# CoderWZW/ARLib

Hardware: AMD Instinct MI355X
Metric: BPR-train interactions/sec (LightGCN d=64 L=3 + BPR + Adam, B=2048) (higher is better)
Workload: dtype f32

## Files before the change

### arlib_amd/_lib.py

```python
import ctypes as C
import os

_HERE = os.path.dirname(os.path.abspath(__file__))
LIB_PATH = os.environ.get('ARLIB_AMD_LIB') or os.path.join(_HERE, 'lib', 'libarlib_amd.so')
ABI_VERSION = 28
_lib = None


class ArlError(RuntimeError):
    pass


class arl_csr(C.Structure):
    _fields_ = [('n_rows', C.c_int64), ('nnz', C.c_int64), ('rowptr', C.c_void_p), ('col', C.c_void_p), ('val', C.c_void_p),
                ('chunk', C.c_int32), ('n_chunks', C.c_int64), ('chunk_row', C.c_void_p), ('chunk_begin', C.c_void_p),
                ('chunk_end', C.c_void_p), ('n_long', C.c_int64), ('long_row', C.c_void_p), ('long_first', C.c_void_p),
                ('long_count', C.c_void_p), ('partial', C.c_void_p), ('row_tasks', C.c_void_p)]


class arl_blocked(C.Structure):
    _fields_ = [('n_waves', C.c_int64), ('rows_per_wave', C.c_int64), ('loads_in_flight', C.c_int64), ('wave_ptr', C.c_void_p), ('wave_rows', C.c_void_p), ('rec_col', C.c_void_p),
                ('rec_val', C.c_void_p), ('n_split', C.c_int64), ('split_row', C.c_void_p), ('split_first', C.c_void_p), ('split_count', C.c_void_p),
                ('partial', C.c_void_p), ('waves_per_group', C.c_int64)]

# ... 6 lines not shown

_vp, _i64, _i32, _f = C.c_void_p, C.c_int64, C.c_int32, C.c_float
_SIGS = {
    'arl_abi_version': (C.c_int, []),
    'arl_mt_seed': (C.c_int, [_vp, _vp, _i64]),
    'arl_sampler_shuffle': (C.c_int, [_vp, _vp, _i64]),
    'arl_mt_sample_range': (C.c_int, [_vp, _i64, _i64, C.c_int32, _vp, _vp]),
    'arl_sampler_next_batch': (C.c_int, [_vp, _vp, _i64, _i64, _i32, _vp, _vp, _i64, _vp, _vp, _vp]),
    'arl_norm_adj_values_f32': (C.c_int, [_i64, _vp, _vp, _vp, _vp, _vp, _vp]),
    'arl_norm_adj_values_coo_f32': (C.c_int, [_i64, _vp, _vp, _vp, _vp, _i64, _vp, _vp, _vp]),
    'arl_norm_vals_coo_f32': (C.c_int, [_vp, _vp, _vp, _i64, _vp, _vp, _vp]),
    'arl_spmm_csr_f32': (C.c_int, [C.POINTER(arl_csr), _vp, _i64, _f, _f, _vp, _vp, _vp]),
    'arl_spmm_csr_layersum_f32': (C.c_int, [C.POINTER(arl_csr), _vp, _i64, _vp, _vp, _vp, _vp]),
    'arl_spmm_csr_adam_f32': (C.c_int, [C.POINTER(arl_csr), _vp, _i64, _f, _f, _vp, _vp, _vp, _vp, _vp, _f, _f, _f, _f, _i64, _vp]),
    'arl_spmm_blocked_f32': (C.c_int, [C.POINTER(arl_blocked), _vp, _i64, _f, _f, _vp, _vp, _vp, _vp]),
    'arl_spmm_csr_rscale_f32': (C.c_int, [C.POINTER(arl_csr), _vp, _i64, _vp, _f, _f, _vp, _vp, _vp]),
    'arl_spmm_blocked_rscale_f32': (C.c_int, [C.POINTER(arl_blocked), _vp, _i64, _vp, _f, _f, _vp, _vp, _vp]),
    'arl_spmm_blocked_layersum_f32': (C.c_int, [C.POINTER(arl_blocked), _vp, _i64, _vp, _vp, _vp, _vp]),
    'arl_spmm_blocked_adam_f32': (C.c_int, [C.POINTER(arl_blocked), _vp, _i64, _f, _f, _vp, _vp, _vp, _vp, _vp, _f, _f, _f, _f, _i64, _vp]),
    'arl_lpt_deal': (C.c_int, [_i64, _vp, _i64, _i64, _vp, _vp]),
    'arl_syn_v1_pairs': (_i64, [_i64, _i64, C.c_double, C.c_uint64, C.c_double, _i64, _i64, _vp, _i64]),
    'arl_graph_digest': (C.c_uint64, [_vp, _i64]),
    'arl_spmm_tiled_f32': (C.c_int, [C.POINTER(arl_tiled), _vp, _i64, _f, _f, _vp, _vp, _vp, _vp]),
    'arl_spmm_tiled_adam_f32': (C.c_int, [C.POINTER(arl_tiled), _vp, _i64, _f, _f, _vp, _vp, _vp, _vp, _vp, _f, _f, _f, _f, _i64, _vp]),
    'arl_spmm_csr_flagged_f32': (C.c_int, [C.POINTER(arl_csr), _vp, _i64, _vp, _f, _f, _vp, _vp, _vp, _vp]),
    'arl_spmm_csr_rows_workspace_bytes': (_i64, [_i64, _i64, _i64]),
    'arl_spmm_csr_rows_f32': (C.c_int, [C.POINTER(arl_csr), _vp, _i64, _vp, _i64, _i64, _vp, _i64, _f, _vp, _vp, _vp, _vp]),
    'arl_mark_rows_u8': (C.c_int, [_vp, _vp, _i64, _i32, _vp]),
    'arl_mark_rows_bits_u32': (C.c_int, [_vp, _vp, _i64, _i32, _vp]),
    'arl_zero_rows_f32': (C.c_int, [_vp, _vp, _i64, _i64, _vp]),
    'arl_batch_rows_set_f32': (C.c_int, [_vp, _vp, _vp, _vp, _i64, _i64, _vp, _f, _vp, _vp, _vp]),
    'arl_batch_rows_clear_f32': (C.c_int, [_vp, _vp, _vp, _vp, _i64, _i64, _vp, _vp]),
    'arl_bpr_l2_workspace_bytes': (_i64, [_i64]),
    'arl_bpr_l2_fwd_bwd_f32': (C.c_int, [_vp, _i64, _i64, _vp, _vp, _vp, _i64, _f, _f, _vp, _vp, _vp, _i32, _vp]),
    'arl_bpr_l2_partial_f32': (C.c_int, [_vp, _i64, _i64, _vp, _vp, _vp, _i64, _i64, _vp, _vp, _vp]),
    'arl_bpr_l2_backward_f32': (C.c_int, [_vp, _i64, _i64, _vp, _vp, _vp, _i64, _f, _f, _vp, _vp, _vp, _vp]),
    'arl_adam_dense_f32': (C.c_int, [_vp, _vp, _vp, _vp, _i64, _f, _f, _f, _f, _i64, _vp]),
    'arl_sgd_dense_f32': (C.c_int, [_vp, _vp, _i64, _f, _vp]),
    'arl_gather_rows_f32': (C.c_int, [_vp, _vp, _i64, _i64, _vp, _vp]),
    'arl_scatter_add_rows_f32': (C.c_int, [_vp, _vp, _i64, _i64, _vp, _f, _vp]),
    'arl_rows_axpy_unique_f32': (C.c_int, [_vp, _vp, _vp, _i64, _i64, _f, _vp, _vp]),
    'arl_shard_batch_prep_i32': (C.c_int, [_vp, _vp, _vp, _i64, _i64, _i64, _vp, _vp, _vp, _vp, _vp]),
# ... 92 lines not shown
```

### arlib_amd/csrc/arl_host.cpp

```cpp
#include <cstdint>
#include <cstddef>
#include <queue>
#include <cmath>
#include <algorithm>
#include <utility>
#include <vector>
#include "arlib_amd.h"

namespace {

class PyMersenne {
public:
    explicit PyMersenne(uint32_t *state) : w_(state), pos_(state[kN]) {}
    ~PyMersenne() { w_[kN] = pos_; }

    uint32_t next32() {
        if (pos_ >= kN) refill();
        uint32_t y = w_[pos_++];
        y ^= y >> 11;
        y ^= (y << 7) & 0x9d2c5680u;
        y ^= (y << 15) & 0xefc60000u;
        return y ^ (y >> 18);
    }

// ... 41 lines not shown

inline bool user_has_item(const int64_t *rowptr, const int32_t *items, int64_t rows, int32_t user, int32_t item) {
    if (user < 0 || user >= rows) return false;
    const int32_t *lo = items + rowptr[user], *hi = items + rowptr[user + 1];
    while (lo < hi) {
        const int32_t *mid = lo + (hi - lo) / 2;
        if (*mid < item) lo = mid + 1; else hi = mid;
    }
    return lo < items + rowptr[user + 1] && *lo == item;
}

}

extern "C" {

int arl_abi_version(void) { return 28; }

int arl_mt_seed(uint32_t *mt_state, const uint32_t *key, int64_t key_len) {
    if (!mt_state || !key) return ARL_E_NULL;
    if (key_len < 1) return ARL_E_ARG;
    PyMersenne::seed_by_array(mt_state, key, key_len);
    return ARL_OK;
}

int arl_sampler_shuffle(uint32_t *mt_state, int32_t *pairs, int64_t nnz) {
    if (!mt_state || (!pairs && nnz > 0)) return ARL_E_NULL;
    if (nnz < 0 || nnz > 0xFFFFFFFFll) return ARL_E_RANGE;
    if (mt_state[624] > 624) return ARL_E_ARG;
    PyMersenne rng(mt_state);
    int64_t *rows = reinterpret_cast<int64_t *>(pairs);
    const bool aligned = (reinterpret_cast<uintptr_t>(pairs) & 7u) == 0;
// ... 148 lines not shown
```

### arlib_amd/csrc/arl_kernels.hip

```cpp
#include <hip/hip_runtime.h>
#include <stdint.h>
#include <math.h>
#include <stdio.h>
#include <stdlib.h>
#include "arlib_amd.h"
#include <type_traits>

#define ARL_LAUNCH_CHECK()                                  \
    do {                                                    \
        hipError_t e__ = hipGetLastError();                 \
        if (e__ != hipSuccess) return (int)e__;             \
    } while (0)

namespace {

constexpr int kWave = 64;
constexpr int kBlock = 256;
constexpr int kWavesPerBlock = kBlock / kWave;

__device__ __forceinline__ float wave_sum(float v) {
#pragma unroll
    for (int off = 32; off > 0; off >>= 1) v += __shfl_xor(v, off);
    return v;
}
// ... 235 lines not shown

template <int LPR>
__global__ __launch_bounds__(kBlock) void subset_finish_kernel(const float *__restrict__ partial, int n, int nsplit, int d, const int32_t *__restrict__ rows,
                                                                LayerPtrs L, float alpha, float *__restrict__ out_c, const float *__restrict__ row_weight) {
    constexpr int G = kWave / LPR;
    const int lane = threadIdx.x & (kWave - 1);
    const int g = lane / LPR, q = lane % LPR;
    const int t = (blockIdx.x * kWavesPerBlock + (threadIdx.x >> 6)) * G + g;
    if (t >= n || q * 4 >= d) return;
    const int r = rows[t];
    float4 a = make_float4(0.f, 0.f, 0.f, 0.f);
    for (int k = 0; k < L.n; ++k) a = add4(a, *reinterpret_cast<const float4 *>(L.p[k] + (size_t)r * d + q * 4));
    for (int s = 0; s < nsplit; ++s) a = add4(a, *reinterpret_cast<const float4 *>(partial + ((size_t)t * nsplit + s) * d + q * 4));
    const float w = row_weight ? alpha * row_weight[t] : alpha;
    *reinterpret_cast<float4 *>(out_c + (size_t)t * d + q * 4) = make_float4(w * a.x, w * a.y, w * a.z, w * a.w);
}

__global__ __launch_bounds__(kBlock) void tables_sum_kernel(LayerPtrs L, long long n4, float alpha, float4 *__restrict__ out) {
    for (long long t = (long long)blockIdx.x * kBlock + threadIdx.x; t < n4; t += (long long)gridDim.x * kBlock) {
        float4 a = reinterpret_cast<const float4 *>(L.p[0])[t];
        for (int k = 1; k < L.n; ++k) a = add4(a, reinterpret_cast<const float4 *>(L.p[k])[t]);
        out[t] = make_float4(alpha * a.x, alpha * a.y, alpha * a.z, alpha * a.w);
    }
}

__global__ __launch_bounds__(kBlock) void mark_rows_kernel(uint8_t *__restrict__ flags, const int32_t *__restrict__ idx, int n, int value) {
    const int t = blockIdx.x * kBlock + threadIdx.x;
    if (t < n) flags[idx[t]] = (uint8_t)value;
}
__global__ __launch_bounds__(kBlock) void mark_bits_kernel(uint32_t *__restrict__ bits, const int32_t *__restrict__ idx, int n, int set) {
// ... 328 lines not shown
    return ARL_OK;
}

typedef float f32x32v __attribute__((ext_vector_type(32)));
#ifndef ARL_SPMM_EXP_NOVAL
#define ARL_SPMM_EXP_NOVAL 0
#endif

struct BlockedDev {
    int n_waves;
    const int32_t *wave_ptr;
    const int32_t *wave_rows;
    const int32_t *rec_col;
    const float *rec_val;
    float *partial;
};

template <int MODE, int CPL, int LD>
__device__ __forceinline__ void spmm_epilogue1(const Epi &ep, int row, int lane, const float *a) {
    const size_t o = (size_t)row * LD + lane * CPL;
    const bool zr = ep.Z && (!ep.zflags || ep.zflags[row]);
#pragma unroll
    for (int c = 0; c < CPL; ++c) {
        if (MODE == EPI_AXPBY) {
            float y = (ep.rscale ? ep.alpha * ep.rscale[row] : ep.alpha) * a[c];
            if (zr) y = fmaf(ep.beta, ep.Z[o + c], y);
            __builtin_nontemporal_store(y, ep.Y + o + c);
        } else if (MODE == EPI_LAYERSUM) {
            const float sv = ep.S_in[o + c];
            if (ep.Y) ep.Y[o + c] = a[c];
            ep.S[o + c] = sv + a[c];
        } else {
            float g = ep.alpha * a[c];
            if (zr) g = fmaf(ep.beta, ep.Z[o + c], g);
            float p = ep.P[o + c], m = ep.M[o + c], v = ep.V[o + c];
            m = m + (g - m) * ep.w1;
            v = v * ep.b2 + ep.w2 * g * g;
            const float denom = sqrtf(v) / ep.bc2_sqrt + ep.eps;
            p = p - ep.step_size * (m / denom);
            ep.P[o + c] = p; ep.M[o + c] = m; ep.V[o + c] = v;
        }
    }
}

template <int RPW, int MODE, int UNR, int CPL, int LD = 64 * CPL>
__global__ __launch_bounds__(kBlock) void spmm_blocked64_kernel(BlockedDev P, const float *__restrict__ X, Epi ep) {
    static_assert(RPW == 16 || RPW == 32, "accumulators are 32-register vectors");
    static_assert(CPL == 1 || CPL == 2, "d = 64 (one column per lane) or d = 128 (two adjacent columns per lane)");
    const int lane = threadIdx.x & 63;
    const int w = blockIdx.x * (blockDim.x >> 6) + (threadIdx.x >> 6);
    if (w >= P.n_waves) return;
    f32x32v acc[CPL];
#pragma unroll
    for (int c = 0; c < CPL; ++c)
#pragma unroll
        for (int r = 0; r < 32; ++r) acc[c][r] = 0.f;
    const int begin = P.wave_ptr[w], end = P.wave_ptr[w + 1];
    const float *xl = X + lane * CPL;
    int rc = 0; float rv = 0.f;
    if (begin < end) { rc = __builtin_nontemporal_load(P.rec_col + begin + lane); if (!ARL_SPMM_EXP_NOVAL) rv = __builtin_nontemporal_load(P.rec_val + begin + lane); }
    for (int base = begin; base < end; base += 64) {
        const int c_cur = rc; const float v_cur = rv;
        if (base + 64 < end) { rc = __builtin_nontemporal_load(P.rec_col + base + 64 + lane); if (!ARL_SPMM_EXP_NOVAL) rv = __builtin_nontemporal_load(P.rec_val + base + 64 + lane); }
#pragma unroll
        for (int j = 0; j < 64; j += UNR) {
            float x[UNR][CPL]; int cs[UNR];
#pragma unroll
            for (int t = 0; t < UNR; ++t) {
                cs[t] = __builtin_amdgcn_readlane(c_cur, j + t);
                const float *src = xl + (size_t)(cs[t] & 0xffffff) * LD;
                if (CPL == 2) { const float2 v2 = *reinterpret_cast<const float2 *>(src); x[t][0] = v2.x; x[t][CPL - 1] = v2.y; }
                else x[t][0] = src[0];
            }
#pragma unroll
            for (int t = 0; t < UNR; ++t) {
                const int slot = ((unsigned)cs[t] >> 24) & 31;
                if (ARL_SPMM_EXP_NOVAL) {
#pragma unroll
                    for (int c = 0; c < CPL; ++c) acc[c][slot] += x[t][c];
                    continue;
                }
                const float v = __uint_as_float((unsigned)__builtin_amdgcn_readlane((int)__float_as_uint(v_cur), j + t));
#pragma unroll
                for (int c = 0; c < CPL; ++c) acc[c][slot] = fmaf(v, x[t][c], acc[c][slot]);
            }
        }
    }
#pragma unroll
    for (int r = 0; r < RPW; ++r) {
        const int row = P.wave_rows[w * RPW + r];
        float a[CPL];
#pragma unroll
        for (int c = 0; c < CPL; ++c) a[c] = acc[c][r];
        if (row >= 0) spmm_epilogue1<MODE, CPL, LD>(ep, row, lane, a);
        else if (row < -1) {
            float *dst = P.partial + ((size_t)(-row - 2) * 64 + lane) * CPL;
#pragma unroll
            for (int c = 0; c < CPL; ++c) dst[c] = a[c];
        }
    }
}

#ifndef ARL_D128_HALF_HOPS
#define ARL_D128_HALF_HOPS 1
#endif
template <int MODE>
int launch_spmm_blocked(const arl_blocked *P, const float *X, int64_t d, const Epi &ep, hipStream_t st) {
    if (!P || !X) return ARL_E_NULL;
    if (d != 64 && d != 128) return ARL_E_DIM;
    if (P->n_waves < 0 || P->n_waves > 0x7fffffffll / 64) return ARL_E_RANGE;
    if (P->rows_per_wave != 16 && P->rows_per_wave != 32) return ARL_E_ARG;
    if (P->n_waves == 0) return ARL_OK;
    if (!P->wave_ptr || !P->wave_rows || !P->rec_col || !P->rec_val) return ARL_E_NULL;
    if (P->n_split < 0 || P->n_split > 0x7fffffffll) return ARL_E_RANGE;
    if (P->n_split > 0 && (!P->split_row || !P->split_first || !P->split_count || !P->partial)) return ARL_E_NULL;
    BlockedDev D = {(int)P->n_waves, P->wave_ptr, P->wave_rows, P->rec_col, P->rec_val, P->partial};
    const int64_t wpg = P->waves_per_group ? P->waves_per_group : kWavesPerBlock;
    if (wpg != 1 && wpg != 2 && wpg != 4) return ARL_E_ARG;
    const dim3 grid((unsigned)((P->n_waves + wpg - 1) / wpg)), block((unsigned)(wpg * kWave));
    if (P->loads_in_flight != 16 && P->loads_in_flight != 32) return ARL_E_ARG;
#if ARL_D128_HALF_HOPS
    if (d == 128) {
        for (int half = 0; half < 2; ++half) {
            Epi e2 = ep;
            e2.ld = 128;
            const int off = 64 * half;
            if (e2.Z) e2.Z += off;
            if (e2.Y) e2.Y += off;
            if (e2.S_in) e2.S_in += off;
            if (e2.S) e2.S += off;
            if (e2.P) e2.P += off;
            if (e2.M) e2.M += off;
            if (e2.V) e2.V += off;
            if (P->rows_per_wave == 16) hipLaunchKernelGGL((spmm_blocked64_kernel<16, MODE, 16, 1, 128>), grid, block, 0, st, D, X + off, e2);
            else if (P->loads_in_flight == 16) hipLaunchKernelGGL((spmm_blocked64_kernel<32, MODE, 16, 1, 128>), grid, block, 0, st, D, X + off, e2);
            else hipLaunchKernelGGL((spmm_blocked64_kernel<32, MODE, 32, 1, 128>), grid, block, 0, st, D, X + off, e2);
            ARL_LAUNCH_CHECK();
            if (P->n_split > 0) {
                CsrDev C = {};
                C.n_long = (int)P->n_split; C.long_row = P->split_row; C.long_first = P->split_first; C.long_count = P->split_count; C.partial = P->partial;
                const unsigned grid_long = (unsigned)((C.n_long + kWavesPerBlock - 1) / kWavesPerBlock);
                hipLaunchKernelGGL((spmm_long_rows_kernel<16, MODE>), dim3(grid_long), dim3(kBlock), 0, st, C, 64, e2);
                ARL_LAUNCH_CHECK();
            }
        }
        return ARL_OK;
    }
#endif
    if (d == 128) {
        if (P->rows_per_wave == 16) hipLaunchKernelGGL((spmm_blocked64_kernel<16, MODE, 16, 2>), grid, block, 0, st, D, X, ep);
        else hipLaunchKernelGGL((spmm_blocked64_kernel<32, MODE, 16, 2>), grid, block, 0, st, D, X, ep);
    } else if (P->rows_per_wave == 16) hipLaunchKernelGGL((spmm_blocked64_kernel<16, MODE, 16, 1>), grid, block, 0, st, D, X, ep);
    else if (P->loads_in_flight == 16) hipLaunchKernelGGL((spmm_blocked64_kernel<32, MODE, 16, 1>), grid, block, 0, st, D, X, ep);
    else hipLaunchKernelGGL((spmm_blocked64_kernel<32, MODE, 32, 1>), grid, block, 0, st, D, X, ep);
    ARL_LAUNCH_CHECK();
    if (P->n_split > 0) {
        CsrDev C = {};
        C.n_long = (int)P->n_split; C.long_row = P->split_row; C.long_first = P->split_first; C.long_count = P->split_count; C.partial = P->partial;
        const unsigned grid_long = (unsigned)((C.n_long + kWavesPerBlock - 1) / kWavesPerBlock);
        if (d == 128) hipLaunchKernelGGL((spmm_long_rows_kernel<32, MODE>), dim3(grid_long), dim3(kBlock), 0, st, C, 128, ep);
        else hipLaunchKernelGGL((spmm_long_rows_kernel<16, MODE>), dim3(grid_long), dim3(kBlock), 0, st, C, 64, ep);
        ARL_LAUNCH_CHECK();
    }
    return ARL_OK;
}

__global__ __launch_bounds__(kBlock) void row_dinv_kernel(int n_rows, const int32_t *__restrict__ rowptr,
                                                           const float *__restrict__ w, float *__restrict__ dinv) {
    const int lane = threadIdx.x & 63;
    const int r = blockIdx.x * kWavesPerBlock + (threadIdx.x >> 6);
// ... 3293 lines not shown
    Epi ep = {};
    ep.S_in = S_in; ep.S = S; ep.Y = Y;
    return launch_spmm<EPI_LAYERSUM>(A, X, d, ep, (hipStream_t)stream);
}

int arl_spmm_blocked_f32(const arl_blocked *P, const float *X, int64_t d, float alpha, float beta, const float *Z, const uint8_t *zflags, float *Y,
                         arl_stream_t stream) {
    if (!Y) return ARL_E_NULL;
    if (beta != 0.f && !Z) return ARL_E_NULL;
    if (Y == X) return ARL_E_ARG;
    Epi ep = {};
    ep.alpha = alpha; ep.beta = beta; ep.Z = (beta != 0.f) ? Z : nullptr; ep.zflags = zflags; ep.Y = Y;
    return launch_spmm_blocked<EPI_AXPBY>(P, X, d, ep, (hipStream_t)stream);
}

int arl_spmm_blocked_rscale_f32(const arl_blocked *P, const float *X, int64_t d, const float *row_scale, float alpha, float beta, const float *Z,
                                float *Y, arl_stream_t stream) {
    if (!Y || !row_scale) return ARL_E_NULL;
    if (beta != 0.f && !Z) return ARL_E_NULL;
    if (Y == X) return ARL_E_ARG;
    Epi ep = {};
    ep.alpha = alpha; ep.beta = beta; ep.Z = (beta != 0.f) ? Z : nullptr; ep.Y = Y; ep.rscale = row_scale;
    return launch_spmm_blocked<EPI_AXPBY>(P, X, d, ep, (hipStream_t)stream);
}

int arl_spmm_blocked_layersum_f32(const arl_blocked *P, const float *X, int64_t d, const float *S_in, float *S, float *Y, arl_stream_t stream) {
    if (!S_in || !S) return ARL_E_NULL;
    if (Y == X) return ARL_E_ARG;
    Epi ep = {};
    ep.S_in = S_in; ep.S = S; ep.Y = Y;
// ... 55 lines not shown
    if (step < 1) return ARL_E_ARG;
    if (P == X) return ARL_E_ARG;
    Epi ep = {};
    ep.alpha = alpha; ep.beta = beta; ep.Z = (beta != 0.f) ? Z : nullptr; ep.zflags = zflags; ep.P = P; ep.M = M; ep.V = V;
    {
        const AdamScalars a = adam_scalars(lr, beta1, beta2, step);
        ep.step_size = a.step_size; ep.bc2_sqrt = a.bc2_sqrt; ep.w1 = a.w1; ep.b2 = a.b2; ep.w2 = a.w2; ep.eps = (float)typed_double(eps);
    }
    return launch_spmm<EPI_ADAM>(A, X, d, ep, (hipStream_t)stream);
}

int64_t arl_spmm_csr_rows_workspace_bytes(int64_t n_rows_sel, int64_t nsplit, int64_t d) {
    return (n_rows_sel < 0 || nsplit < 1 || d < 0) ? 0 : (int64_t)sizeof(float) * n_rows_sel * nsplit * d;
}

int arl_spmm_csr_rows_f32(const arl_csr *A, const float *X, int64_t d, const int32_t *rows, int64_t n_rows_sel, int64_t nsplit,
                          const float *const *layers, int64_t n_layers, float alpha, const float *row_weight, float *out_c, void *workspace,
                          arl_stream_t stream) {
    if (!A || !X || !rows || !out_c || !workspace || !A->rowptr) return ARL_E_NULL;
    if (A->nnz > 0 && (!A->col || !A->val)) return ARL_E_NULL;
    if (n_layers < 0 || n_layers > 8 || (n_layers > 0 && !layers)) return ARL_E_ARG;
    if (d <= 0 || d > 256 || (d & 3)) return ARL_E_DIM;
    if (n_rows_sel < 0 || nsplit < 1 || nsplit > 1024 || n_rows_sel * nsplit > 0x7fffffffll) return ARL_E_RANGE;
    if (n_rows_sel == 0) return ARL_OK;
    hipStream_t st = (hipStream_t)stream;
    CsrDev D = {};
    D.n_rows = (int)A->n_rows; D.rowptr = A->rowptr; D.col = A->col; D.val = A->val;
    LayerPtrs LP = {};
    LP.n = (int)n_layers;
    for (int k = 0; k < LP.n; ++k) { if (!layers[k]) return ARL_E_NULL; LP.p[k] = layers[k]; }
    const long long tasks = n_rows_sel * nsplit;
    const unsigned grid = (unsigned)((tasks + kWavesPerBlock - 1) / kWavesPerBlock);
    const int di = (int)d, n = (int)n_rows_sel, ns = (int)nsplit;
    float *part = (float *)workspace;
#define ARL_SUBSET_CASE(LPRV)                                                                                                  \
    do {                                                                                                                       \
        hipLaunchKernelGGL((spmm_subset_kernel<LPRV>), dim3(grid), dim3(kBlock), 0, st, D, X, di, rows, n, ns, part);          \
        ARL_LAUNCH_CHECK();                                                                                                    \
        const unsigned g2 = (unsigned)((n + kWavesPerBlock * (kWave / LPRV) - 1) / (kWavesPerBlock * (kWave / LPRV)));         \
        hipLaunchKernelGGL((subset_finish_kernel<LPRV>), dim3(g2), dim3(kBlock), 0, st, part, n, ns, di, rows, LP, alpha, out_c, row_weight); \
        ARL_LAUNCH_CHECK();                                                                                                    \
    } while (0)
    if (d <= 16) ARL_SUBSET_CASE(4);
    else if (d <= 32) ARL_SUBSET_CASE(8);
    else if (d <= 64) ARL_SUBSET_CASE(16);
    else if (d <= 128) ARL_SUBSET_CASE(32);
    else ARL_SUBSET_CASE(64);
#undef ARL_SUBSET_CASE
    return ARL_OK;
}

int arl_mark_rows_u8(uint8_t *flags, const int32_t *idx, int64_t n, int32_t value, arl_stream_t stream) {
    if (!flags || !idx) return ARL_E_NULL;
    if (n < 0 || n > 0x7fffffffll) return ARL_E_ARG;
    if (n == 0) return ARL_OK;
    hipLaunchKernelGGL(mark_rows_kernel, dim3((unsigned)((n + kBlock - 1) / kBlock)), dim3(kBlock), 0, (hipStream_t)stream, flags, idx, (int)n, (int)value);
    ARL_LAUNCH_CHECK();
    return ARL_OK;
}

int arl_mark_rows_bits_u32(uint32_t *bits, const int32_t *idx, int64_t n, int32_t set, arl_stream_t stream) {
    if (!bits || !idx) return ARL_E_NULL;
    if (n < 0 || n > 0x7fffffffll) return ARL_E_ARG;
    if (n == 0) return ARL_OK;
// ... 1049 lines not shown
```

### arlib_amd/ops.py

```python
import ctypes as C
import os
import time
import numpy as np
import torch

from . import _lib
from ._lib import arl_csr, check

DEFAULT_CHUNK = 512
EVENT_HOOK = None


_raw_stream = getattr(torch._C, '_cuda_getCurrentRawStream', None)


def _stream():
    if _raw_stream is not None:
        return C.c_void_p(_raw_stream(torch.cuda.current_device()))
    return C.c_void_p(torch.cuda.current_stream().cuda_stream)


def _dev(t, dtype, name, ndim=None):
    if not isinstance(t, torch.Tensor):
        raise TypeError('%s: expected a torch.Tensor' % name)
# ... 608 lines not shown
    Y = torch.empty(A.n_rows, d, dtype=torch.float32, device=X.device) if out is None else out
    if _check_xy(A, Y, 'out') != d or Y.data_ptr() == X.data_ptr():
        raise ValueError('spmm_flagged: out must be [n_rows, d] and must not alias X')
    if beta != 0.0 and (Z is None or _check_xy(A, Z, 'Z') != d):
        raise ValueError('spmm_flagged: Z [n_rows, d] required when beta != 0')
    if xflags is not None:
        _dev(xflags, torch.int32, 'xflags (bitmap)', 1)
        if xflags.numel() != (A.n_cols + 31) // 32:
            raise ValueError('spmm_flagged: bitmap needs ceil(n_cols/32) int32 words')
    if zflags is not None:
        _check_flags(zflags, A.n_rows, 'zflags')
    L, zp, st = _lib.lib(), (_ptr(Z) if beta != 0.0 else None), _stream()
    tok = EVENT_HOOK.begin('masked' if xflags is not None else 'axpby') if EVENT_HOOK is not None else None
    csr = lambda p: check(L.arl_spmm_csr_flagged_f32(p, _ptr(X), d, _ptr(xflags), alpha, beta, zp, _ptr(zflags), _ptr(Y), st), 'arl_spmm_csr_flagged_f32')
    if xflags is not None:
        csr(C.byref(A._struct(d)))
    else:
        _spmm_dispatch(A, d, lambda p: check(L.arl_spmm_blocked_f32(p, _ptr(X), d, alpha, beta, zp, _ptr(zflags), _ptr(Y), st), 'arl_spmm_blocked_f32'), csr)
    if tok is not None:
        EVENT_HOOK.end(tok)
    return Y


ROWS_NSPLIT = 16


def spmm_rows(A, X, rows, layers=(), alpha=1.0, nsplit=ROWS_NSPLIT, out=None, workspace=None, check_range=True, row_weight=None):
    d = _check_xy(A, X, 'X', A.n_cols)
    _dev(rows, torch.int32, 'rows', 1)
    n = rows.numel()
    if check_range and n and (int(rows.min()) < 0 or int(rows.max()) >= A.n_rows):
        raise IndexError('spmm_rows: row index out of range')
    if len(layers) > 8:
        raise ValueError('spmm_rows: at most 8 layer tables')
    for t in layers:
        if _check_xy(A, t, 'layer') != d:
            raise ValueError('spmm_rows: layer table shape mismatch')
    if out is None:
        out = torch.empty(n, d, dtype=torch.float32, device=X.device)
    _dev(out, torch.float32, 'out', 2)
    if out.shape != (n, d):
        raise ValueError('spmm_rows: out must be [len(rows), d]')
    need = _lib.lib().arl_spmm_csr_rows_workspace_bytes(n, nsplit, d) // 4
    if workspace is None or workspace.numel() < need:
        workspace = torch.empty(max(need, 1), dtype=torch.float32, device=X.device)
    arr = (C.c_void_p * max(len(layers), 1))(*[t.data_ptr() for t in layers])
    s = A._struct(d)
    tok = EVENT_HOOK.begin('rows') if EVENT_HOOK is not None else None
    if row_weight is not None and (_dev(row_weight, torch.float32, 'row_weight', 1).numel() != n):
        raise ValueError('spmm_rows: row_weight must have one entry per listed row')
    check(_lib.lib().arl_spmm_csr_rows_f32(C.byref(s), _ptr(X), d, _ptr(rows), n, nsplit, C.cast(arr, C.c_void_p), len(layers), alpha, _ptr(row_weight),
                                           _ptr(out), _ptr(workspace), _stream()), 'arl_spmm_csr_rows_f32')
    if tok is not None:
        EVENT_HOOK.end(tok)
    return out


def mark_rows_(flags, idx, value, check_range=True):
    _dev(flags, torch.uint8, 'flags', 1); _dev(idx, torch.int32, 'idx', 1)
    if check_range and idx.numel() and (int(idx.min()) < 0 or int(idx.max()) >= flags.numel()):
        raise IndexError('mark_rows_: index out of range')
    check(_lib.lib().arl_mark_rows_u8(_ptr(flags), _ptr(idx), idx.numel(), int(value), _stream()), 'arl_mark_rows_u8')
    return flags


def batch_rows_set_(G, flags, bits, idx, src, scale=1.0, check_range=True, row_scale=None, dup_bits=None):
    _dev(G, torch.float32, 'G', 2); _dev(flags, torch.uint8, 'flags', 1); _dev(bits, torch.int32, 'bits', 1); _dev(idx, torch.int32, 'idx', 1)
# ... 1143 lines not shown
```

### include/arlib_amd.h

```cpp
#ifndef ARLIB_AMD_H
#define ARLIB_AMD_H

#include <stdint.h>

#ifdef __cplusplus
extern "C" {
#endif

#define ARL_OK 0
#define ARL_E_NULL (-1)
#define ARL_E_DIM (-2)
#define ARL_E_RANGE (-3)
#define ARL_E_ARG (-4)

typedef void *arl_stream_t;

int arl_abi_version(void);

int arl_mt_seed(uint32_t *mt_state, const uint32_t *key, int64_t key_len);
int arl_sampler_shuffle(uint32_t *mt_state, int32_t *pairs, int64_t nnz);
int arl_mt_sample_range(uint32_t *mt_state, int64_t n, int64_t k, int32_t use_pool, int32_t *out, int32_t *scratch);
int arl_sampler_next_batch(uint32_t *mt_state, const int32_t *pairs, int64_t begin, int64_t count,
                           int32_t n_items, const int64_t *memb_rowptr, const int32_t *memb_items,
                           int64_t memb_rows, int32_t *out_u, int32_t *out_p, int32_t *out_n);
// ... 26 lines not shown

int arl_spmm_csr_f32(const arl_csr *A, const float *X, int64_t d, float alpha, float beta, const float *Z,
                     float *Y, arl_stream_t stream);
int arl_spmm_csr_layersum_f32(const arl_csr *A, const float *X, int64_t d, const float *S_in, float *S,
                              float *Y, arl_stream_t stream);
int arl_spmm_csr_adam_f32(const arl_csr *A, const float *X, int64_t d, float alpha, float beta, const float *Z,
                          const uint8_t *zflags, float *P, float *M, float *V, float lr, float beta1, float beta2,
                          float eps, int64_t step, arl_stream_t stream);

int arl_spmm_csr_flagged_f32(const arl_csr *A, const float *X, int64_t d, const uint32_t *xbits, float alpha, float beta,
                             const float *Z, const uint8_t *zflags, float *Y, arl_stream_t stream);
int64_t arl_spmm_csr_rows_workspace_bytes(int64_t n_rows_sel, int64_t nsplit, int64_t d);
int arl_spmm_csr_rows_f32(const arl_csr *A, const float *X, int64_t d, const int32_t *rows, int64_t n_rows_sel,
                          int64_t nsplit, const float *const *layers, int64_t n_layers, float alpha, const float *row_weight,
                          float *out_c, void *workspace, arl_stream_t stream);
int arl_mark_rows_u8(uint8_t *flags, const int32_t *idx, int64_t n, int32_t value, arl_stream_t stream);
int arl_mark_rows_bits_u32(uint32_t *bits, const int32_t *idx, int64_t n, int32_t set, arl_stream_t stream);
int arl_zero_rows_f32(float *dst, const int32_t *idx, int64_t n, int64_t d, arl_stream_t stream);
int arl_batch_rows_set_f32(float *G, uint8_t *flags, uint32_t *bits, const int32_t *idx, int64_t n, int64_t d,
                           const float *src, float scale, const float *row_scale, uint32_t *dup_bits, arl_stream_t stream);
int arl_batch_rows_clear_f32(float *G, uint8_t *flags, uint32_t *bits, const int32_t *idx, int64_t n, int64_t d,
                             uint32_t *dup_bits, arl_stream_t stream);

typedef struct arl_blocked {
    int64_t n_waves, rows_per_wave;
    int64_t loads_in_flight;
    const int32_t *wave_ptr;
    const int32_t *wave_rows;
    const int32_t *rec_col;
    const float *rec_val;
    int64_t n_split;
    const int32_t *split_row;
    const int32_t *split_first;
    const int32_t *split_count;
    float *partial;
    int64_t waves_per_group;
} arl_blocked;
int arl_spmm_blocked_f32(const arl_blocked *P, const float *X, int64_t d, float alpha, float beta, const float *Z,
                         const uint8_t *zflags, float *Y, arl_stream_t stream);
int arl_spmm_csr_rscale_f32(const arl_csr *A, const float *X, int64_t d, const float *row_scale, float alpha, float beta,
                            const float *Z, float *Y, arl_stream_t stream);
int arl_spmm_blocked_rscale_f32(const arl_blocked *P, const float *X, int64_t d, const float *row_scale, float alpha,
                                float beta, const float *Z, float *Y, arl_stream_t stream);
int arl_spmm_blocked_layersum_f32(const arl_blocked *P, const float *X, int64_t d, const float *S_in, float *S, float *Y,
                                  arl_stream_t stream);
int arl_spmm_blocked_adam_f32(const arl_blocked *P, const float *X, int64_t d, float alpha, float beta, const float *Z,
                              const uint8_t *zflags, float *Pm, float *M, float *V, float lr, float beta1, float beta2,
                              float eps, int64_t step, arl_stream_t stream);
int arl_lpt_deal(int64_t n, const int32_t *weight_desc, int64_t n_bins, int64_t cap, int32_t *bin_out, int32_t *slot_out);

int64_t arl_syn_v1_pairs(int64_t n_users, int64_t n_items, double mean_deg, uint64_t seed, double sigma, int64_t deg_min, int64_t deg_max,
                         int32_t *pairs_out, int64_t capacity);
uint64_t arl_graph_digest(const int32_t *pairs, int64_t n);

// ... 160 lines not shown
```

Baseline: 320,600.

## Add masked blocked SpMM and edge-piece load balancing for row-subset SpMM

Adds a masked variant of the blocked 64-wide SpMM that checks a column bitmask and only gathers the columns whose bit is set, and routes the flagged SpMM in Python to it instead of the CSR flagged kernel. It also changes the row-subset SpMM so that each selected row is split into fixed-size edge pieces. A single-block prep kernel builds the piece plan, then a pieces kernel and a finish reduction run, replacing the fixed nsplit partition. The aim is to cut wasted gathers on sparse masks and to even out load across rows of very different degree, at the cost of an extra prep launch and a serial one-block planning step.

```diff
diff --git a/arlib_amd/_lib.py b/arlib_amd/_lib.py
--- a/arlib_amd/_lib.py
+++ b/arlib_amd/_lib.py
@@ -3,7 +3,7 @@
 
 _HERE = os.path.dirname(os.path.abspath(__file__))
 LIB_PATH = os.environ.get('ARLIB_AMD_LIB') or os.path.join(_HERE, 'lib', 'libarlib_amd.so')
-ABI_VERSION = 28
+ABI_VERSION = 29
 _lib = None
 
 
@@ -44,6 +44,7 @@
     'arl_spmm_csr_layersum_f32': (C.c_int, [C.POINTER(arl_csr), _vp, _i64, _vp, _vp, _vp, _vp]),
     'arl_spmm_csr_adam_f32': (C.c_int, [C.POINTER(arl_csr), _vp, _i64, _f, _f, _vp, _vp, _vp, _vp, _vp, _f, _f, _f, _f, _i64, _vp]),
     'arl_spmm_blocked_f32': (C.c_int, [C.POINTER(arl_blocked), _vp, _i64, _f, _f, _vp, _vp, _vp, _vp]),
+    'arl_spmm_blocked_flagged_f32': (C.c_int, [C.POINTER(arl_blocked), _vp, _i64, _vp, _f, _f, _vp, _vp, _vp, _vp]),
     'arl_spmm_csr_rscale_f32': (C.c_int, [C.POINTER(arl_csr), _vp, _i64, _vp, _f, _f, _vp, _vp, _vp]),
     'arl_spmm_blocked_rscale_f32': (C.c_int, [C.POINTER(arl_blocked), _vp, _i64, _vp, _f, _f, _vp, _vp, _vp]),
     'arl_spmm_blocked_layersum_f32': (C.c_int, [C.POINTER(arl_blocked), _vp, _i64, _vp, _vp, _vp, _vp]),
@@ -56,6 +57,8 @@
     'arl_spmm_csr_flagged_f32': (C.c_int, [C.POINTER(arl_csr), _vp, _i64, _vp, _f, _f, _vp, _vp, _vp, _vp]),
     'arl_spmm_csr_rows_workspace_bytes': (_i64, [_i64, _i64, _i64]),
     'arl_spmm_csr_rows_f32': (C.c_int, [C.POINTER(arl_csr), _vp, _i64, _vp, _i64, _i64, _vp, _i64, _f, _vp, _vp, _vp, _vp]),
+    'arl_spmm_csr_rows_pieces_f32': (C.c_int, [C.POINTER(arl_csr), _vp, _i64, _vp, _i64, _i64, _i64, _vp, _i64, _f, _vp, _vp, _vp, _vp]),
+    'arl_spmm_csr_rows_scratch_offset': (_i64, [_i64, _i64, _i64]),
     'arl_mark_rows_u8': (C.c_int, [_vp, _vp, _i64, _i32, _vp]),
     'arl_mark_rows_bits_u32': (C.c_int, [_vp, _vp, _i64, _i32, _vp]),
     'arl_zero_rows_f32': (C.c_int, [_vp, _vp, _i64, _i64, _vp]),
diff --git a/arlib_amd/csrc/arl_host.cpp b/arlib_amd/csrc/arl_host.cpp
--- a/arlib_amd/csrc/arl_host.cpp
+++ b/arlib_amd/csrc/arl_host.cpp
@@ -79,7 +79,7 @@
 
 extern "C" {
 
-int arl_abi_version(void) { return 28; }
+int arl_abi_version(void) { return 29; }
 
 int arl_mt_seed(uint32_t *mt_state, const uint32_t *key, int64_t key_len) {
     if (!mt_state || !key) return ARL_E_NULL;
diff --git a/arlib_amd/csrc/arl_kernels.hip b/arlib_amd/csrc/arl_kernels.hip
--- a/arlib_amd/csrc/arl_kernels.hip
+++ b/arlib_amd/csrc/arl_kernels.hip
@@ -273,6 +273,132 @@
     for (int s = 0; s < nsplit; ++s) a = add4(a, *reinterpret_cast<const float4 *>(partial + ((size_t)t * nsplit + s) * d + q * 4));
     const float w = row_weight ? alpha * row_weight[t] : alpha;
     *reinterpret_cast<float4 *>(out_c + (size_t)t * d + q * 4) = make_float4(w * a.x, w * a.y, w * a.z, w * a.w);
+}
+
+constexpr int kSubsetPieceEdges = 1024;
+constexpr int kSubsetPrepThreads = 1024;
+constexpr int kSubsetPrepRows = 8;
+constexpr int kSubsetMaxWaves = 16384;
+
+struct SubsetPlan {
+    int cap;
+    int32_t *piece_row;
+    int32_t *meta;
+    int32_t *offs;
+};
+
+__global__ __launch_bounds__(kSubsetPrepThreads) void subset_prep_kernel(const int32_t *__restrict__ rowptr, const int32_t *__restrict__ rows, int n, int piece_edges,
+                                                                          SubsetPlan S) {
+    constexpr int NW = kSubsetPrepThreads / kWave, R = kSubsetPrepRows;
+    __shared__ long long wsum[NW];
+    const int tid = threadIdx.x, lane = tid & (kWave - 1), wv = tid >> 6;
+    const int per = (n + kSubsetPrepThreads - 1) / kSubsetPrepThreads;
+    const int lo = min(n, tid * per), hi = min(n, lo + per);
+    int len[R];
+    {
+        int r[R];
+#pragma unroll
+        for (int k = 0; k < R; ++k) r[k] = lo + k < hi ? rows[lo + k] : -1;
+#pragma unroll
+        for (int k = 0; k < R; ++k) len[k] = r[k] >= 0 ? rowptr[r[k] + 1] - rowptr[r[k]] : -1;
+    }
+    auto pieces_of = [](int l, unsigned P) { return (unsigned)l > P ? ((unsigned)l + P - 1u) / P : 1u; };
+    unsigned P = (unsigned)piece_edges;
+    long long mine, incl, total;
+    for (;;) {
+        mine = 0;
+#pragma unroll
+        for (int k = 0; k < R; ++k) if (len[k] >= 0) mine += pieces_of(len[k], P);
+        incl = mine;
+#pragma unroll
+        for (int off = 1; off < kWave; off <<= 1) { const long long o = __shfl_up(incl, off); if (lane >= off) incl += o; }
+        __syncthreads();
+        if (lane == kWave - 1) wsum[wv] = incl;
+        __syncthreads();
+        total = 0;
+        long long before = 0;
+#pragma unroll
+        for (int k = 0; k < NW; ++k) { const long long v = wsum[k]; total += v; if (k < wv) before += v; }
+        incl += before;
+        if (total <= S.cap) break;
+        P *= 2;
+    }
+    int first = (int)(incl - mine);
+#pragma unroll
+    for (int k = 0; k < R; ++k) {
+        const int t = lo + k;
+        const int sp = len[k] >= 0 ? (int)pieces_of(len[k], P) : 0;
+        if (sp > 0) S.offs[t] = first;
+        if (sp == 1) S.piece_row[first] = t;
+        for (unsigned long long many = __ballot(sp > 1); many; many &= many - 1ull) {
+            const int l = __builtin_ctzll(many);
+            const int sp_l = __builtin_amdgcn_readlane(sp, l), first_l = __builtin_amdgcn_readlane(first, l), t_l = __builtin_amdgcn_readlane(t, l);
+            for (int i = lane; i < sp_l; i += kWave) S.piece_row[first_l + i] = t_l;
+        }
+        first += sp;
+    }
+    if (tid == 0) { S.meta[0] = (int)min(P, 0x7fffffffu); S.meta[1] = (int)total; S.offs[n] = (int)total; }
+}
+
+template <int LPR>
+__global__ __launch_bounds__(kBlock) void spmm_subset_pieces_kernel(CsrDev A, const float *__restrict__ X, int d, const int32_t *__restrict__ rows, SubsetPlan S,
+                                                                     float *__restrict__ partial) {
+    const int lane = threadIdx.x & (kWave - 1), q = lane % LPR;
+    const int total = S.meta[1], n_waves = gridDim.x * kWavesPerBlock;
+    for (int piece = blockIdx.x * kWavesPerBlock + (threadIdx.x >> 6); piece < total; piece += n_waves) {
+        const int t = S.piece_row[piece];
+        const int k = piece - S.offs[t], sp = S.offs[t + 1] - S.offs[t];
+        const int r = rows[t];
+        const int begin = A.rowptr[r], end = A.rowptr[r + 1];
+        const int per = (end - begin + sp - 1) / sp;
+        const int b = begin + k * per, e = min(end, b + per);
+        float4 a = make_float4(0.f, 0.f, 0.f, 0.f);
+        if (b < e) a = spmm_gather<LPR, 4>(A.col, A.val, b, e, X, d, lane);
+        a = group_reduce<LPR>(a);
+        if (lane < LPR && q * 4 < d) *reinterpret_cast<float4 *>(partial + (size_t)piece * d + q * 4) = a;
+    }
+}
+
+template <int LPR>
+__global__ __launch_bounds__(kBlock) void subset_pieces_finish_kernel(const float *__restrict__ partial, int n, SubsetPlan S, int d, const int32_t *__restrict__ rows,
+                                                                       LayerPtrs L, float alpha, float *__restrict__ out_c, const float *__restrict__ row_weight) {
+    constexpr int G = kWave / LPR;
+    const int lane = threadIdx.x & (kWave - 1);
+    const int g = lane / LPR, q = lane % LPR;
+    const int t = blockIdx.x * kWavesPerBlock + (threadIdx.x >> 6);
+    if (t >= n) return;
+    const bool qact = q * 4 < d;
+    const int r = rows[t];
+    float4 a = make_float4(0.f, 0.f, 0.f, 0.f);
+    if (g == 0 && qact)
+        for (int k = 0; k < L.n; ++k) a = add4(a, *reinterpret_cast<const float4 *>(L.p[k] + (size_t)r * d + q * 4));
+    const int p1 = S.offs[t + 1];
+    if (qact)
+        for (int p = S.offs[t] + g; p < p1; p += 8 * G) {
+            float4 v[8];
+#pragma unroll
+            for (int u = 0; u < 8; ++u)
+                if (p + u * G < p1) v[u] = *reinterpret_cast<const float4 *>(partial + (size_t)(p + u * G) * d + q * 4);
+#pragma unroll
+            for (int u = 0; u < 8; ++u)
+                if (p + u * G < p1) a = add4(a, v[u]);
+        }
+    a = group_reduce<LPR>(a);
+    if (lane >= LPR || !qact) return;
+    const float w = row_weight ? alpha * row_weight[t] : alpha;
+    *reinterpret_cast<float4 *>(out_c + (size_t)t * d + q * 4) = make_float4(w * a.x, w * a.y, w * a.z, w * a.w);
+}
+
+static bool subset_plan(void *workspace, long long n, long long nsplit, long long d, SubsetPlan *S) {
+    const long long words = n * nsplit * d, tail = n + 3;
+    const long long cap = (words - tail) / (d + 1);
+    if (cap < n || cap > 0x7fffffffll || n > (long long)kSubsetPrepThreads * kSubsetPrepRows) return false;
+    int32_t *w = (int32_t *)workspace;
+    S->cap = (int)cap;
+    S->piece_row = w + cap * d;
+    S->meta = S->piece_row + cap;
+    S->offs = S->meta + 2;
+    return true;
 }
 
 __global__ __launch_bounds__(kBlock) void tables_sum_kernel(LayerPtrs L, long long n4, float alpha, float4 *__restrict__ out) {
@@ -631,6 +757,7 @@
     const int32_t *rec_col;
     const float *rec_val;
     float *partial;
+    const uint32_t *xbits;
 };
 
 template <int MODE, int CPL, int LD>
@@ -660,7 +787,9 @@
     }
 }
 
-template <int RPW, int MODE, int UNR, int CPL, int LD = 64 * CPL>
+constexpr int kMaskedUnr = 8;
+
+template <int RPW, int MODE, int UNR, int CPL, int LD = 64 * CPL, bool MASKED = false>
 __global__ __launch_bounds__(kBlock) void spmm_blocked64_kernel(BlockedDev P, const float *__restrict__ X, Epi ep) {
     static_assert(RPW == 16 || RPW == 32, "accumulators are 32-register vectors");
     static_assert(CPL == 1 || CPL == 2, "d = 64 (one column per lane) or d = 128 (two adjacent columns per lane)");
@@ -674,6 +803,40 @@
         for (int r = 0; r < 32; ++r) acc[c][r] = 0.f;
     const int begin = P.wave_ptr[w], end = P.wave_ptr[w + 1];
     const float *xl = X + lane * CPL;
+    if (MASKED) {
+        int c0 = 0, c1 = 0; unsigned w0 = 0;
+        if (begin < end) c0 = __builtin_nontemporal_load(P.rec_col + begin + lane);
+        if (begin + 64 < end) c1 = __builtin_nontemporal_load(P.rec_col + begin + 64 + lane);
+        if (begin < end) w0 = P.xbits[((unsigned)c0 & 0xffffffu) >> 5];
+        for (int base = begin; base < end; base += 64) {
+            const int c_cur = c0; const unsigned w_cur = w0;
+            c0 = c1;
+            if (base + 128 < end) c1 = __builtin_nontemporal_load(P.rec_col + base + 128 + lane);
+            if (base + 64 < end) w0 = P.xbits[((unsigned)c0 & 0xffffffu) >> 5];
+            unsigned long long hits = __ballot((w_cur >> (c_cur & 31)) & 1u);
+            while (hits) {
+                float x[kMaskedUnr][CPL], vs[kMaskedUnr]; int cs[kMaskedUnr], js[kMaskedUnr];
+#pragma unroll
+                for (int t = 0; t < kMaskedUnr; ++t) {
+                    js[t] = hits ? __builtin_ctzll(hits) : -1;
+                    hits &= hits - 1ull;
+                    if (js[t] < 0) continue;
+                    cs[t] = __builtin_amdgcn_readlane(c_cur, js[t]);
+                    vs[t] = P.rec_val[base + js[t]];
+                    const float *src = xl + (size_t)(cs[t] & 0xffffff) * LD;
+                    if (CPL == 2) { const float2 v2 = *reinterpret_cast<const float2 *>(src); x[t][0] = v2.x; x[t][CPL - 1] = v2.y; }
+                    else x[t][0] = src[0];
+                }
+#pragma unroll
+                for (int t = 0; t < kMaskedUnr; ++t) {
+                    if (js[t] < 0) continue;
+                    const int slot = ((unsigned)cs[t] >> 24) & 31;
+#pragma unroll
+                    for (int c = 0; c < CPL; ++c) acc[c][slot] = fmaf(vs[t], x[t][c], acc[c][slot]);
+                }
+            }
+        }
+    } else {
     int rc = 0; float rv = 0.f;
     if (begin < end) { rc = __builtin_nontemporal_load(P.rec_col + begin + lane); if (!ARL_SPMM_EXP_NOVAL) rv = __builtin_nontemporal_load(P.rec_val + begin + lane); }
     for (int base = begin; base < end; base += 64) {
@@ -703,6 +866,7 @@
             }
         }
     }
+    }
 #pragma unroll
     for (int r = 0; r < RPW; ++r) {
         const int row = P.wave_rows[w * RPW + r];
@@ -721,8 +885,18 @@
 #ifndef ARL_D128_HALF_HOPS
 #define ARL_D128_HALF_HOPS 1
 #endif
+template <int RPW, int MODE, int UNR, int CPL, int LD>
+static int launch_blocked64(dim3 grid, dim3 block, hipStream_t st, const BlockedDev &D, const float *X, const Epi &ep) {
+    if (D.xbits) {
+        if constexpr (MODE == EPI_AXPBY) hipLaunchKernelGGL((spmm_blocked64_kernel<RPW, MODE, UNR, CPL, LD, true>), grid, block, 0, st, D, X, ep);
+        else return ARL_E_ARG;
+    } else hipLaunchKernelGGL((spmm_blocked64_kernel<RPW, MODE, UNR, CPL, LD, false>), grid, block, 0, st, D, X, ep);
+    ARL_LAUNCH_CHECK();
+    return ARL_OK;
+}
+
 template <int MODE>
-int launch_spmm_blocked(const arl_blocked *P, const float *X, int64_t d, const Epi &ep, hipStream_t st) {
+int launch_spmm_blocked(const arl_blocked *P, const float *X, int64_t d, const Epi &ep, hipStream_t st, const uint32_t *xbits = nullptr) {
     if (!P || !X) return ARL_E_NULL;
     if (d != 64 && d != 128) return ARL_E_DIM;
     if (P->n_waves < 0 || P->n_waves > 0x7fffffffll / 64) return ARL_E_RANGE;
@@ -731,11 +905,12 @@
     if (!P->wave_ptr || !P->wave_rows || !P->rec_col || !P->rec_val) return ARL_E_NULL;
     if (P->n_split < 0 || P->n_split > 0x7fffffffll) return ARL_E_RANGE;
     if (P->n_split > 0 && (!P->split_row || !P->split_first || !P->split_count || !P->partial)) return ARL_E_NULL;
-    BlockedDev D = {(int)P->n_waves, P->wave_ptr, P->wave_rows, P->rec_col, P->rec_val, P->partial};
+    BlockedDev D = {(int)P->n_waves, P->wave_ptr, P->wave_rows, P->rec_col, P->rec_val, P->partial, xbits};
     const int64_t wpg = P->waves_per_group ? P->waves_per_group : kWavesPerBlock;
     if (wpg != 1 && wpg != 2 && wpg != 4) return ARL_E_ARG;
     const dim3 grid((unsigned)((P->n_waves + wpg - 1) / wpg)), block((unsigned)(wpg * kWave));
     if (P->loads_in_flight != 16 && P->loads_in_flight != 32) return ARL_E_ARG;
+    int rc;
 #if ARL_D128_HALF_HOPS
     if (d == 128) {
         for (int half = 0; half < 2; ++half) {
@@ -749,10 +924,10 @@
             if (e2.P) e2.P += off;
             if (e2.M) e2.M += off;
             if (e2.V) e2.V += off;
-            if (P->rows_per_wave == 16) hipLaunchKernelGGL((spmm_blocked64_kernel<16, MODE, 16, 1, 128>), grid, block, 0, st, D, X + off, e2);
-            else if (P->loads_in_flight == 16) hipLaunchKernelGGL((spmm_blocked64_kernel<32, MODE, 16, 1, 128>), grid, block, 0, st, D, X + off, e2);
-            else hipLaunchKernelGGL((spmm_blocked64_kernel<32, MODE, 32, 1, 128>), grid, block, 0, st, D, X + off, e2);
-            ARL_LAUNCH_CHECK();
+            if (P->rows_per_wave == 16) rc = launch_blocked64<16, MODE, 16, 1, 128>(grid, block, st, D, X + off, e2);
+            else if (P->loads_in_flight == 16) rc = launch_blocked64<32, MODE, 16, 1, 128>(grid, block, st, D, X + off, e2);
+            else rc = launch_blocked64<32, MODE, 32, 1, 128>(grid, block, st, D, X + off, e2);
+            if (rc != ARL_OK) return rc;
             if (P->n_split > 0) {
                 CsrDev C = {};
                 C.n_long = (int)P->n_split; C.long_row = P->split_row; C.long_first = P->split_first; C.long_count = P->split_count; C.partial = P->partial;
@@ -765,12 +940,12 @@
     }
 #endif
     if (d == 128) {
-        if (P->rows_per_wave == 16) hipLaunchKernelGGL((spmm_blocked64_kernel<16, MODE, 16, 2>), grid, block, 0, st, D, X, ep);
-        else hipLaunchKernelGGL((spmm_blocked64_kernel<32, MODE, 16, 2>), grid, block, 0, st, D, X, ep);
-    } else if (P->rows_per_wave == 16) hipLaunchKernelGGL((spmm_blocked64_kernel<16, MODE, 16, 1>), grid, block, 0, st, D, X, ep);
-    else if (P->loads_in_flight == 16) hipLaunchKernelGGL((spmm_blocked64_kernel<32, MODE, 16, 1>), grid, block, 0, st, D, X, ep);
-    else hipLaunchKernelGGL((spmm_blocked64_kernel<32, MODE, 32, 1>), grid, block, 0, st, D, X, ep);
-    ARL_LAUNCH_CHECK();
+        if (P->rows_per_wave == 16) rc = launch_blocked64<16, MODE, 16, 2, 128>(grid, block, st, D, X, ep);
+        else rc = launch_blocked64<32, MODE, 16, 2, 128>(grid, block, st, D, X, ep);
+    } else if (P->rows_per_wave == 16) rc = launch_blocked64<16, MODE, 16, 1, 64>(grid, block, st, D, X, ep);
+    else if (P->loads_in_flight == 16) rc = launch_blocked64<32, MODE, 16, 1, 64>(grid, block, st, D, X, ep);
+    else rc = launch_blocked64<32, MODE, 32, 1, 64>(grid, block, st, D, X, ep);
+    if (rc != ARL_OK) return rc;
     if (P->n_split > 0) {
         CsrDev C = {};
         C.n_long = (int)P->n_split; C.long_row = P->split_row; C.long_first = P->split_first; C.long_count = P->split_count; C.partial = P->partial;
@@ -4094,6 +4269,16 @@
     return launch_spmm_blocked<EPI_AXPBY>(P, X, d, ep, (hipStream_t)stream);
 }
 
+int arl_spmm_blocked_flagged_f32(const arl_blocked *P, const float *X, int64_t d, const uint32_t *xbits, float alpha, float beta, const float *Z,
+                                 const uint8_t *zflags, float *Y, arl_stream_t stream) {
+    if (!Y || !xbits) return ARL_E_NULL;
+    if (beta != 0.f && !Z) return ARL_E_NULL;
+    if (Y == X) return ARL_E_ARG;
+    Epi ep = {};
+    ep.alpha = alpha; ep.beta = beta; ep.Z = (beta != 0.f) ? Z : nullptr; ep.zflags = zflags; ep.Y = Y;
+    return launch_spmm_blocked<EPI_AXPBY>(P, X, d, ep, (hipStream_t)stream, xbits);
+}
+
 int arl_spmm_blocked_rscale_f32(const arl_blocked *P, const float *X, int64_t d, const float *row_scale, float alpha, float beta, const float *Z,
                                 float *Y, arl_stream_t stream) {
     if (!Y || !row_scale) return ARL_E_NULL;
@@ -4179,9 +4364,16 @@
     return (n_rows_sel < 0 || nsplit < 1 || d < 0) ? 0 : (int64_t)sizeof(float) * n_rows_sel * nsplit * d;
 }
 
-int arl_spmm_csr_rows_f32(const arl_csr *A, const float *X, int64_t d, const int32_t *rows, int64_t n_rows_sel, int64_t nsplit,
-                          const float *const *layers, int64_t n_layers, float alpha, const float *row_weight, float *out_c, void *workspace,
-                          arl_stream_t stream) {
+int64_t arl_spmm_csr_rows_scratch_offset(int64_t n_rows_sel, int64_t nsplit, int64_t d) {
+    SubsetPlan S = {};
+    if (n_rows_sel <= 0 || nsplit < 1 || nsplit > 1024 || d <= 0 || d > 256 || (d & 3) || !subset_plan(nullptr, n_rows_sel, nsplit, d, &S)) return -1;
+    return (int64_t)S.cap * (d + 1);
+}
+
+int arl_spmm_csr_rows_pieces_f32(const arl_csr *A, const float *X, int64_t d, const int32_t *rows, int64_t n_rows_sel, int64_t nsplit, int64_t piece_edges,
+                                 const float *const *layers, int64_t n_layers, float alpha, const float *row_weight, float *out_c, void *workspace,
+                                 arl_stream_t stream) {
+    if (piece_edges < 0 || piece_edges > 0x40000000ll) return ARL_E_RANGE;
     if (!A || !X || !rows || !out_c || !workspace || !A->rowptr) return ARL_E_NULL;
     if (A->nnz > 0 && (!A->col || !A->val)) return ARL_E_NULL;
     if (n_layers < 0 || n_layers > 8 || (n_layers > 0 && !layers)) return ARL_E_ARG;
@@ -4198,8 +4390,22 @@
     const unsigned grid = (unsigned)((tasks + kWavesPerBlock - 1) / kWavesPerBlock);
     const int di = (int)d, n = (int)n_rows_sel, ns = (int)nsplit;
     float *part = (float *)workspace;
+    SubsetPlan S = {};
+    const bool pieces = subset_plan(workspace, n_rows_sel, nsplit, d, &S);
+    if (pieces) {
+        hipLaunchKernelGGL(subset_prep_kernel, dim3(1), dim3(kSubsetPrepThreads), 0, st, A->rowptr, rows, n, piece_edges > 0 ? (int)piece_edges : kSubsetPieceEdges, S);
+        ARL_LAUNCH_CHECK();
+    }
+    const unsigned grid_p = (unsigned)(((S.cap < kSubsetMaxWaves ? S.cap : kSubsetMaxWaves) + kWavesPerBlock - 1) / kWavesPerBlock);
 #define ARL_SUBSET_CASE(LPRV)                                                                                                  \
     do {                                                                                                                       \
+        if (pieces) {                                                                                                          \
+            hipLaunchKernelGGL((spmm_subset_pieces_kernel<LPRV>), dim3(grid_p), dim3(kBlock), 0, st, D, X, di, rows, S, part); \
+            ARL_LAUNCH_CHECK();                                                                                                \
+            hipLaunchKernelGGL((subset_pieces_finish_kernel<LPRV>), dim3((unsigned)((n + kWavesPerBlock - 1) / kWavesPerBlock)), dim3(kBlock), 0, st, part, n, S, di, rows, LP, alpha, out_c, row_weight); \
+            ARL_LAUNCH_CHECK();                                                                                                \
+            break;                                                                                                             \
+        }                                                                                                                      \
         hipLaunchKernelGGL((spmm_subset_kernel<LPRV>), dim3(grid), dim3(kBlock), 0, st, D, X, di, rows, n, ns, part);          \
         ARL_LAUNCH_CHECK();                                                                                                    \
         const unsigned g2 = (unsigned)((n + kWavesPerBlock * (kWave / LPRV) - 1) / (kWavesPerBlock * (kWave / LPRV)));         \
@@ -4213,6 +4419,12 @@
     else ARL_SUBSET_CASE(64);
 #undef ARL_SUBSET_CASE
     return ARL_OK;
+}
+
+int arl_spmm_csr_rows_f32(const arl_csr *A, const float *X, int64_t d, const int32_t *rows, int64_t n_rows_sel, int64_t nsplit,
+                          const float *const *layers, int64_t n_layers, float alpha, const float *row_weight, float *out_c, void *workspace,
+                          arl_stream_t stream) {
+    return arl_spmm_csr_rows_pieces_f32(A, X, d, rows, n_rows_sel, nsplit, 0, layers, n_layers, alpha, row_weight, out_c, workspace, stream);
 }
 
 int arl_mark_rows_u8(uint8_t *flags, const int32_t *idx, int64_t n, int32_t value, arl_stream_t stream) {
diff --git a/arlib_amd/ops.py b/arlib_amd/ops.py
--- a/arlib_amd/ops.py
+++ b/arlib_amd/ops.py
@@ -646,7 +646,8 @@
     tok = EVENT_HOOK.begin('masked' if xflags is not None else 'axpby') if EVENT_HOOK is not None else None
     csr = lambda p: check(L.arl_spmm_csr_flagged_f32(p, _ptr(X), d, _ptr(xflags), alpha, beta, zp, _ptr(zflags), _ptr(Y), st), 'arl_spmm_csr_flagged_f32')
     if xflags is not None:
-        csr(C.byref(A._struct(d)))
+        _spmm_dispatch(A, d, lambda p: check(L.arl_spmm_blocked_flagged_f32(p, _ptr(X), d, _ptr(xflags), alpha, beta, zp, _ptr(zflags), _ptr(Y), st),
+                                             'arl_spmm_blocked_flagged_f32'), csr)
     else:
         _spmm_dispatch(A, d, lambda p: check(L.arl_spmm_blocked_f32(p, _ptr(X), d, alpha, beta, zp, _ptr(zflags), _ptr(Y), st), 'arl_spmm_blocked_f32'), csr)
     if tok is not None:
@@ -657,7 +658,16 @@
 ROWS_NSPLIT = 16
 
 
-def spmm_rows(A, X, rows, layers=(), alpha=1.0, nsplit=ROWS_NSPLIT, out=None, workspace=None, check_range=True, row_weight=None):
+def spmm_rows_plan(left_in, n, nsplit, d):
+    off = _lib.lib().arl_spmm_csr_rows_scratch_offset(n, nsplit, d)
+    if off < 0:
+        return None
+    w = left_in.view(torch.int32)
+    meta = w[off:off + 2].tolist()
+    return meta[0], meta[1], w[off + 2:off + 3 + n]
+
+
+def spmm_rows(A, X, rows, layers=(), alpha=1.0, nsplit=ROWS_NSPLIT, out=None, workspace=None, check_range=True, row_weight=None, piece_edges=0):
     d = _check_xy(A, X, 'X', A.n_cols)
     _dev(rows, torch.int32, 'rows', 1)
     n = rows.numel()
@@ -681,8 +691,12 @@
     tok = EVENT_HOOK.begin('rows') if EVENT_HOOK is not None else None
     if row_weight is not None and (_dev(row_weight, torch.float32, 'row_weight', 1).numel() != n):
         raise ValueError('spmm_rows: row_weight must have one entry per listed row')
-    check(_lib.lib().arl_spmm_csr_rows_f32(C.byref(s), _ptr(X), d, _ptr(rows), n, nsplit, C.cast(arr, C.c_void_p), len(layers), alpha, _ptr(row_weight),
-                                           _ptr(out), _ptr(workspace), _stream()), 'arl_spmm_csr_rows_f32')
+    if piece_edges:
+        check(_lib.lib().arl_spmm_csr_rows_pieces_f32(C.byref(s), _ptr(X), d, _ptr(rows), n, nsplit, int(piece_edges), C.cast(arr, C.c_void_p), len(layers), alpha,
+                                                      _ptr(row_weight), _ptr(out), _ptr(workspace), _stream()), 'arl_spmm_csr_rows_pieces_f32')
+    else:
+        check(_lib.lib().arl_spmm_csr_rows_f32(C.byref(s), _ptr(X), d, _ptr(rows), n, nsplit, C.cast(arr, C.c_void_p), len(layers), alpha, _ptr(row_weight),
+                                               _ptr(out), _ptr(workspace), _stream()), 'arl_spmm_csr_rows_f32')
     if tok is not None:
         EVENT_HOOK.end(tok)
     return out
diff --git a/include/arlib_amd.h b/include/arlib_amd.h
--- a/include/arlib_amd.h
+++ b/include/arlib_amd.h
@@ -64,6 +64,10 @@
 int arl_spmm_csr_rows_f32(const arl_csr *A, const float *X, int64_t d, const int32_t *rows, int64_t n_rows_sel,
                           int64_t nsplit, const float *const *layers, int64_t n_layers, float alpha, const float *row_weight,
                           float *out_c, void *workspace, arl_stream_t stream);
+int arl_spmm_csr_rows_pieces_f32(const arl_csr *A, const float *X, int64_t d, const int32_t *rows, int64_t n_rows_sel,
+                                 int64_t nsplit, int64_t piece_edges, const float *const *layers, int64_t n_layers, float alpha,
+                                 const float *row_weight, float *out_c, void *workspace, arl_stream_t stream);
+int64_t arl_spmm_csr_rows_scratch_offset(int64_t n_rows_sel, int64_t nsplit, int64_t d);
 int arl_mark_rows_u8(uint8_t *flags, const int32_t *idx, int64_t n, int32_t value, arl_stream_t stream);
 int arl_mark_rows_bits_u32(uint32_t *bits, const int32_t *idx, int64_t n, int32_t set, arl_stream_t stream);
 int arl_zero_rows_f32(float *dst, const int32_t *idx, int64_t n, int64_t d, arl_stream_t stream);
@@ -88,6 +92,8 @@
 } arl_blocked;
 int arl_spmm_blocked_f32(const arl_blocked *P, const float *X, int64_t d, float alpha, float beta, const float *Z,
                          const uint8_t *zflags, float *Y, arl_stream_t stream);
+int arl_spmm_blocked_flagged_f32(const arl_blocked *P, const float *X, int64_t d, const uint32_t *xbits, float alpha, float beta,
+                                 const float *Z, const uint8_t *zflags, float *Y, arl_stream_t stream);
 int arl_spmm_csr_rscale_f32(const arl_csr *A, const float *X, int64_t d, const float *row_scale, float alpha, float beta,
                             const float *Z, float *Y, arl_stream_t stream);
 int arl_spmm_blocked_rscale_f32(const arl_blocked *P, const float *X, int64_t d, const float *row_scale, float alpha,
```

New measurement: 327,500, median of 6. 1.02x the previous value.
